# ManuelWendl/Monocular_Visual_Odometry_VA4MR

Measured on AMD Instinct MI355X. Metric: frames/s + ATE vs ref, KITTI seq00 1241x376 @ 1/2/4/8 MI355X, higher is better.
Workload: dtype mixed(u8,i32,f32,f64)

## Files before the change

### include/vo_hip.h

```cpp
#ifndef VO_HIP_H
#define VO_HIP_H
#include <stdint.h>

#ifdef __cplusplus
extern "C" {
#endif

typedef void* vo_stream_t;

enum vo_err {
    VO_OK = 0,
    VO_EARG = -1,
    VO_EHIP = -2,
};

enum vo_chain_status {
    VO_ST_OK = 0,
    VO_ST_NOT_ENOUGH_KP = 1,
    VO_ST_PNP_FAILED = 2,
    VO_ST_GFTT_NONE = 3,
    VO_ST_GFTT_ONE = 4,
    VO_ST_CAPACITY = 5,
    VO_ST_ESSENTIAL_FAILED = 6,
    VO_ST_NO_MATCHES = 7,
};

#define VO_MAX_LEVELS 8
#define VO_BORDER 16

typedef struct vo_dims {
    int32_t B, W, H;
    int32_t nlev;
    int32_t lvl_w[VO_MAX_LEVELS], lvl_h[VO_MAX_LEVELS], lvl_pitch[VO_MAX_LEVELS];
    int64_t lvl_off[VO_MAX_LEVELS];
    int64_t pyr_stride;
    int64_t der_stride;
    int32_t ncap, pcap, fcap;
    int32_t ccap;
    int32_t mcap;
    int64_t work_stride;
    int64_t iwork_stride;
} vo_dims;

typedef struct vo_opts {
    double K[9], K_inv[9];
    double min_dist_landmarks, max_dist_landmarks;
    double min_baseline_angle;
    double cos_baseline;
    int32_t min_baseline_frames;
    double feature_ratio;
    int32_t feature_max_corners;
    double feature_quality_level, feature_min_dist;
    int32_t feature_block_size, feature_use_harris;
    double harris_k;
    int32_t win_w, win_h, max_level, crit_type, crit_count;
    double crit_eps;
    double min_eig;
    double pnp_conf, pnp_error;
    int32_t pnp_iters;
} vo_opts;

typedef struct vo_state {
    uint8_t* pyr[2];
    int16_t* der[2];
// ... 237 lines not shown
```

### monocular_visual_odometry_va4mr_amd/_lib.py

```python
from __future__ import annotations

import ctypes as C
import os
import subprocess

_HERE = os.path.dirname(os.path.abspath(__file__))
LIB_PATH = os.environ.get("VO_HIP_LIB") or os.path.join(_HERE, "_build", "libvo_hip.so")
CSRC = os.path.join(_HERE, "csrc")

VO_MAX_LEVELS = 8
VO_BORDER = 16
VO_LK_USE_INITIAL_FLOW = 4
VO_LK_GET_MIN_EIGENVALS = 8
VO_LK_ILLUM_BIAS = 1
VO_LK_ILLUM_GAIN_BIAS = 2

ST_OK = 0
ST_NOT_ENOUGH_KP = 1
ST_PNP_FAILED = 2
ST_GFTT_NONE = 3
ST_GFTT_ONE = 4
ST_CAPACITY = 5
ST_ESSENTIAL_FAILED = 6
ST_NO_MATCHES = 7

STATUS_NAMES = {
    ST_OK: "ok",
    ST_NOT_ENOUGH_KP: "Not enough keypoints for PnP",
    ST_PNP_FAILED: "PnP failed",
    ST_GFTT_NONE: "goodFeaturesToTrack returned no corners",
    ST_GFTT_ONE: "goodFeaturesToTrack returned a single corner",
    ST_CAPACITY: "engine capacity exceeded",
    ST_ESSENTIAL_FAILED: "findEssentialMat found no model",
    ST_NO_MATCHES: "no bootstrap matches",
}

i32, i64, f64, vp = C.c_int32, C.c_int64, C.c_double, C.c_void_p


class VoDims(C.Structure):
    _fields_ = [
        ("B", i32), ("W", i32), ("H", i32), ("nlev", i32),
        ("lvl_w", i32 * VO_MAX_LEVELS), ("lvl_h", i32 * VO_MAX_LEVELS), ("lvl_pitch", i32 * VO_MAX_LEVELS),
        ("lvl_off", i64 * VO_MAX_LEVELS),
        ("pyr_stride", i64), ("der_stride", i64),
        ("ncap", i32), ("pcap", i32), ("fcap", i32), ("ccap", i32), ("mcap", i32),
        ("work_stride", i64), ("iwork_stride", i64),
    ]


class VoOpts(C.Structure):
    _fields_ = [
        ("K", f64 * 9), ("K_inv", f64 * 9),
        ("min_dist_landmarks", f64), ("max_dist_landmarks", f64),
        ("min_baseline_angle", f64), ("cos_baseline", f64),
        ("min_baseline_frames", i32),
        ("feature_ratio", f64),
        ("feature_max_corners", i32),
        ("feature_quality_level", f64), ("feature_min_dist", f64),
        ("feature_block_size", i32), ("feature_use_harris", i32),
        ("harris_k", f64),
        ("win_w", i32), ("win_h", i32), ("max_level", i32), ("crit_type", i32), ("crit_count", i32),
        ("crit_eps", f64), ("min_eig", f64),
        ("pnp_conf", f64), ("pnp_error", f64),
        ("pnp_iters", i32),
    ]


_STATE_FIELDS = [
    "pyr0", "pyr1", "der0", "der1", "lm_X", "lm_kp", "nL", "c_kp", "c_first", "c_tau", "nC",
# ... 142 lines not shown
```

### monocular_visual_odometry_va4mr_amd/csrc/vo_lk.hip

```cpp
#include "vo_dev.h"

#include <float.h>
#include <math.h>
#include <type_traits>

namespace {

struct LKParams {
    const uint8_t* prev;
    const int16_t* der;
    const uint8_t* next;
    int64_t pstride, dstride;
    int L;
    int lw[VO_MAX_LEVELS], lh[VO_MAX_LEVELS], lpitch[VO_MAX_LEVELS];
    int64_t loff[VO_MAX_LEVELS];
    int win_w, win_h, max_count;
    double eps2;
    float min_eig;
    float eps2_lo, eps2_hi;
    const float* p0;
    const int32_t* n0;
    int cap0;
    const float* p1;
    const int32_t* n1;
    int cap1;
    int seg1_min;
    const int32_t* chain_status;
    float* out;
    uint8_t* st;
    float* err;
    int ocap;
    const float* init;
    int eig_err;
    const float* fwd;
    double thr2;
};

VO_DEV bool lk_block(int B, int nb, int& b, int& pb, bool xcd = true, int L = -1)
{
    if (L < 0) L = blockIdx.x;
    if (B >= 8 && xcd) {
        const int xcd = L & 7, k = L >> 3;
        b = xcd + 8 * (k / nb);
        pb = k % nb;
    } else {
        b = L / nb;
        pb = L % nb;
    }
    return b < B;
}

#define LK_M 4
VO_DEV __amdgpu_buffer_rsrc_t lkq_rsrc(const void* base, int64_t bytes)
{
    return __builtin_amdgcn_make_buffer_rsrc((void*)base, (short)0, (int)bytes, 0x00020000);
}
#ifndef LK_JPRE
#define LK_JPRE 1
// ... 362 lines not shown
#endif
#ifdef VO_LK_PROF
#define LKPROF_T(var) const long long var = wall_clock64()
#else
#define LKPROF_T(var) do { } while (0)
#endif

#ifdef VO_LK_CHECK
#define LKCHK(ptr, base, bytes, what) \
    (((const char*)(ptr) >= (const char*)(base) && (const char*)(ptr) + 4 <= (const char*)(base) + (bytes)) ? true : \
     (printf("LKCHK %s b=%d p=%d level=%d off=%lld size=%lld\n", what, b, pcur, level, \
             (long long)((const char*)(ptr) - (const char*)(base)), (long long)(bytes)), false))
#else
#define LKCHK(ptr, base, bytes, what) true
#endif
#ifdef VO_LK_CHECK
#define LKCHKO(off, bytes, what) \
    do { if ((off) < 0 || (int64_t)(off) + 4 > (int64_t)(bytes)) \
        printf("LKCHK %s b=%d p=%d level=%d off=%lld size=%lld\n", what, b, pcur, level, (long long)(off), (long long)(bytes)); } while (0)
#else
#define LKCHKO(off, bytes, what) do { } while (0)
#endif

template <int WW, int WH, bool EX = false, bool ERR = true>
__global__ void __launch_bounds__(64) __attribute__((amdgpu_waves_per_eu(8, 8))) k_lk_w(LKParams P, int level_hi, int level_lo, int B, int nb, int xcd)
{
    constexpr int WPB = 1;
    constexpr int NPX = WW * WH, MAXJ = (NPX + 63) / 64;
    constexpr int TW = WW + 2 * LK_M, TH = WH + 2 * LK_M;
    constexpr int JRW = (TW + 1 + 3 + 3) / 4, IRW = (WW + 1 + 3 + 3) / 4, DRW = WW + 1;
    constexpr int QM = (TW + 3) / 4, QS = 4 * QM;
    constexpr int IRS = QS / 4, JRS = 8;
    static_assert(JRW >= QM + 1 && JRW <= JRS && IRW <= IRS && IRW <= 8 && DRW == 16 && QS % 4 == 0,
                  "k_lk_w staging layout");
    __shared__ uint4 QT4_all[WPB][(TH + 1) * QM];
    __shared__ uint32_t IR_all[WPB][(WH + 2) * IRS];
    __shared__ uint32_t DR_all[WPB][(WH + 2) * QS];
    const int wv = WPB > 1 ? (int)(threadIdx.x >> 6) : 0;
    uint4* QT4 = QT4_all[wv];
    const uint32_t* QT = reinterpret_cast<const uint32_t*>(QT4);
    uint32_t* IR = IR_all[wv];
    uint32_t* DR = DR_all[wv];
    const uint8_t* ir8 = (const uint8_t*)IR;
    int b, pb, pcur = -1;
    const int lane = lane_id();
    int level = level_lo;
    LKPROF_SET(0, wall_clock64()); LKPROF_SET(1, 0);
    for (level = level_hi; level >= level_lo; --level)
        for (int k = 2; k < 8; ++k) LKPROF_SET(k, 0);
    level = level_lo;
    if (!lk_block(B, nb, b, pb, xcd != 0, (int)blockIdx.x * WPB + wv)) return;
    if (P.chain_status && P.chain_status[b] != 0) return;
    const int n0 = P.n0 ? P.n0[b] : 0;
    int n1 = P.n1 ? P.n1[b] : 0;
    if (n1 <= P.seg1_min) n1 = 0;
    const int ntot = n0 + n1;
    const float hx = (WW - 1) * 0.5f, hy = (WH - 1) * 0.5f;
    double eps2;
    asm volatile("" : "=s"(eps2) : "0"(P.eps2));
    float eps2_lo, eps2_hi;
// ... 106 lines not shown
                    oy = __int_as_float(__builtin_amdgcn_readfirstlane(__float_as_int(P.init[2 * oidx + 1]))) * sc;
                }
            }
        }
        else if (level == level_hi) {
            ox = __int_as_float(__builtin_amdgcn_readfirstlane(__float_as_int(P.out[2 * oidx]))) * 2.f;
            oy = __int_as_float(__builtin_amdgcn_readfirstlane(__float_as_int(P.out[2 * oidx + 1]))) * 2.f;
        } else {
            ox *= 2.f;
            oy *= 2.f;
        }
        px -= hx;
        py -= hy;
        const int ipx = (int)floorf(px), ipy = (int)floorf(py);
        do {
            if ((unsigned)(ipx + WW) >= colsW || (unsigned)(ipy + WH) >= rowsW) {
                if (level == 0) { status = 0; errv = 0.f; }
                break;
            }
            bool staged = false;
            {
                LKPROF_T(ti0);
                const int gx = ipx + VO_BORDER, gy = ipy + VO_BORDER;
                const int ish = gx & 3;
                const int ln = lane;
                const int vi = loff + gy * pitch + (gx & ~3) + (ln >> 3) * pitch + 4 * (ln & 7);
                const int drow = 2 * ((ln >> 4) & 1) + (ln >> 5);
                const int vd = 4 * (loff + gy * pitch + gx + drow * pitch + (ln & 15));
                uint32_t vir[NIR], vdd[NDR], vjr[2][NJR];
#pragma unroll
                for (int k = 0; k < NIR; ++k) {
                    LKCHKO(vi + 8 * k * pitch, P.pstride, "I");
                    vir[k] = __builtin_amdgcn_raw_buffer_load_b32(rI, vi, 8 * k * pitch, 0);
                }
#pragma unroll
                for (int k = 0; k < NDR; ++k) {
                    LKCHKO(vd + 16 * k * pitch, 2 * P.dstride, "D");
                    vdd[k] = __builtin_amdgcn_raw_buffer_load_b32(rD, vd, 16 * k * pitch, 0);
                }
                {
                    const int jx = (int)floorf(ox - hx), jy = (int)floorf(oy - hy);
                    staged = LK_JPRE && (unsigned)(jx + WW) < colsW && (unsigned)(jy + WH) < rowsW && P.max_count > 0;
                    if (staged) {
                        LKPROF_ADD(3, 1);
                        j_origin(jx, jy);
                        j_issue(vjr);
                    } else {
                        tx0 = ty0 = -(1 << 28);
                    }
                }
                wave_lds_sync();
#pragma unroll
                for (int k = 0; k < NIR; ++k) {
                    const int r = (ln >> 3) + 8 * k, c = ln & 7;
                    if (c < IRS) IR[r * IRS + c] = vir[k];
                }
#pragma unroll
                for (int k = 0; k < NDR; ++k) {
                    const int r = drow + 4 * k, c = ln & 15;
                    DR[r * QS + c] = vdd[k];
                }
                if (staged) j_store(vjr);
                else wave_lds_sync();
                LKPROF_T(ti1);
                LKPROF_ADD(4, ti1 - ti0);
                float a = px - ipx, bb = py - ipy;
                const int iw00 = __float2int_rn((1.f - a) * (1.f - bb) * (float)(1 << 14));
                const int iw01 = __float2int_rn(a * (1.f - bb) * (float)(1 << 14));
                const int iw10 = __float2int_rn((1.f - a) * bb * (float)(1 << 14));
                const int iw11 = (1 << 14) - iw00 - iw01 - iw10;
                int ival[MAXJ], ixv[MAXJ], iyv[MAXJ];
                uint32_t iseed[MAXJ];
                int a11 = 0, a12 = 0, a22 = 0;
                const v2i16 wp0 = as_v2i16((uint32_t)(iw00 & 0xffff) | ((uint32_t)iw01 << 16));
                const v2i16 wp1 = as_v2i16((uint32_t)(iw10 & 0xffff) | ((uint32_t)iw11 << 16));
#pragma unroll
                for (int j = 0; j < MAXJ; ++j) {
                    const uint8_t* s = ir8 + toff[j] + ish;
                    const uint32_t* d = DR + toff[j];
                    const uint32_t d00 = d[0], d01 = d[1], d10 = d[QS], d11 = d[QS + 1];
                    const int v = DESCALE(__mul24((int)s[0], iw00) + __mul24((int)s[1], iw01) +
                                          __mul24((int)s[QS], iw10) + __mul24((int)s[QS + 1], iw11), 9);
                    const int gx2 = __builtin_amdgcn_sdot2(as_v2i16(__builtin_amdgcn_perm(d11, d10, 0x05040100u)), wp1,
                                        sdot2_sacc(__builtin_amdgcn_perm(d01, d00, 0x05040100u), v2u(wp0), 1 << 13),
                                        false) >> 14;
                    const int gy2 = __builtin_amdgcn_sdot2(as_v2i16(__builtin_amdgcn_perm(d11, d10, 0x07060302u)), wp1,
                                        sdot2_sacc(__builtin_amdgcn_perm(d01, d00, 0x07060302u), v2u(wp0), 1 << 13),
                                        false) >> 14;
                    ival[j] = v;
                    iseed[j] = 256u - ((uint32_t)ival[j] << 9);
                    ixv[j] = live[j] ? gx2 : 0;
                    iyv[j] = live[j] ? gy2 : 0;
                }
                const v2i16 gxp0 = as_v2i16(__builtin_amdgcn_perm((uint32_t)ixv[1], (uint32_t)ixv[0], 0x05040100u));
                const v2i16 gxp1 = as_v2i16(__builtin_amdgcn_perm((uint32_t)ixv[3], (uint32_t)ixv[2], 0x05040100u));
                const v2i16 gyp0 = as_v2i16(__builtin_amdgcn_perm((uint32_t)iyv[1], (uint32_t)iyv[0], 0x05040100u));
                const v2i16 gyp1 = as_v2i16(__builtin_amdgcn_perm((uint32_t)iyv[3], (uint32_t)iyv[2], 0x05040100u));
                a11 = __builtin_amdgcn_sdot2(gxp0, gxp0, sdot2_0(v2u(gxp1), v2u(gxp1)), false);
                a12 = __builtin_amdgcn_sdot2(gxp0, gyp0, sdot2_sacc(v2u(gxp1), v2u(gyp1), 1 << 24), false);
                a22 = __builtin_amdgcn_sdot2(gyp0, gyp0, sdot2_0(v2u(gyp1), v2u(gyp1)), false);
                const bool twide = __ballot(max(max((uint32_t)a11, (uint32_t)a22), (uint32_t)a12) >= (1u << 25)) != 0;
// ... 177 lines not shown
    }
    P.win_w = o->win_w;
    P.win_h = o->win_h;
    int mc = o->crit_count;
    double eps = o->crit_eps;
    if (!(o->crit_type & 1)) mc = 30;
    else mc = mc < 0 ? 0 : (mc > 100 ? 100 : mc);
    if (!(o->crit_type & 2)) eps = 0.01;
    else eps = eps < 0 ? 0 : (eps > 10 ? 10 : eps);
    P.max_count = mc;
    P.eps2 = eps * eps;
    P.min_eig = (float)o->min_eig;
    if (P.eps2 >= 0x1p-100 && P.eps2 <= 0x1p100) {
        P.eps2_lo = nextafterf((float)(P.eps2 * (1. - 0x1p-20)), 0.f);
        P.eps2_hi = nextafterf((float)(P.eps2 * (1. + 0x1p-20)), INFINITY);
    } else {
        P.eps2_lo = -INFINITY;
        P.eps2_hi = INFINITY;
    }
    P.init = nullptr;
    P.eig_err = 0;
    P.fwd = nullptr;
    P.thr2 = 0.;
}

template <bool EX, int ILL = 0>
static int launch_lk_t(const LKParams& P, int B, hipStream_t st)
{
    static_assert(EX || ILL == 0, "the illumination model lives in the EX instantiations");
    const int npx = P.win_w * P.win_h;
    if (P.win_w <= 2 || P.win_h <= 2 || P.win_w > 32 || P.win_h > 32 || npx > 64 * 16 || B < 1) return VO_EARG;
    static const int nb_env = vo_env_int("VO_LK_NB", 0);
    static const int xcd_env = vo_env_int("VO_LK_XCD", 0);
    const int nb = nb_env > 0 ? nb_env : 2048;
    const int nblk = (B >= 8 ? ((B + 7) / 8) * 8 : B) * nb;
    const int L = P.L;
    const int64_t pyr_end = P.loff[L] + (int64_t)(P.lh[L] + 2 * VO_BORDER) * P.lpitch[L];
    const bool staged15 = ILL == 0 && P.win_w == 15 && P.win_h == 15 && P.pstride >= pyr_end + 64;
    const size_t lds = 4 * (size_t)(P.win_w + 2 * LK_M) * (P.win_h + 2 * LK_M);
    if (lds > 60 * 1024) return VO_EARG;
    if (staged15) {
        if (EX || P.err) hipLaunchKernelGGL((k_lk_w<15, 15, EX>), dim3(nblk), dim3(64), 0, st, P, L, 0, B, nb, xcd_env);
        else hipLaunchKernelGGL((k_lk_w<15, 15, false, false>), dim3(nblk), dim3(64), 0, st, P, L, 0, B, nb, xcd_env);
        return hip_ok() ? VO_OK : VO_EHIP;
    }
    const bool big = P.win_w > VO_BORDER || P.win_h > VO_BORDER;
    for (int level = P.L; level >= 0; --level) {
        if (npx > 256) hipLaunchKernelGGL((k_lk<16, true, EX, ILL>), dim3(nblk), dim3(64), lds, st, P, level, B, nb);
        else if (big) hipLaunchKernelGGL((k_lk<4, true, EX, ILL>), dim3(nblk), dim3(64), lds, st, P, level, B, nb);
        else hipLaunchKernelGGL((k_lk<4, false, EX, ILL>), dim3(nblk), dim3(64), lds, st, P, level, B, nb);
    }
    return hip_ok() ? VO_OK : VO_EHIP;
}

static int launch_lk(const LKParams& P, int B, hipStream_t st) { return launch_lk_t<false>(P, B, st); }

static int launch_lk_illum(const LKParams& P, int B, hipStream_t st, int illum)
{
    if (illum == VO_LK_ILLUM_BIAS) return launch_lk_t<true, VO_LK_ILLUM_BIAS>(P, B, st);
    if (illum == VO_LK_ILLUM_GAIN_BIAS) return launch_lk_t<true, VO_LK_ILLUM_GAIN_BIAS>(P, B, st);
    return illum == 0 ? launch_lk_t<true>(P, B, st) : VO_EARG;
}

static bool lk_window_ok(const vo_opts* o)
{
// ... 187 lines not shown
```

### monocular_visual_odometry_va4mr_amd/csrc/vo_pyr.hip

```cpp
#include "vo_dev.h"

namespace {


#define PT_W 128
#define PT_H 16
#ifndef PYR0_TH
#define PYR0_TH 32
#endif
#define PV_W (PT_W + 8)
#define PV_H (PT_H + 2)
#define PS_H (2 * PV_H + 3)
#define PS_W ((2 * PV_W + 3 + 8 + 3) / 4 * 4)

struct PyrLevelArgs {
    const uint8_t* src;
    int64_t sstride;
    int sw, sh, spitch;
    int64_t soff;
    uint8_t* pyr;
    int64_t pstride;
    int16_t* der;
    int64_t dstride;
    int w, h, pitch;
// ... 165 lines not shown
                const int t0l = (ul + ll) * 3 + cl * 10;
                const int t0r = (ur + lr) * 3 + cr * 10;
                dx = t0r - t0l;
                dy = ((lr - ur) + (ll - ul)) * 3 + (lc - uc) * 10;
            }
            o[i] = (uint32_t)(uint16_t)(int16_t)dx | ((uint32_t)(uint16_t)(int16_t)dy << 16);
        }
        int16_t* dq = A.der + (int64_t)b * A.dstride + 2 * (A.off + (int64_t)py * A.pitch + px);
        *(uint4*)dq = make_uint4(o[0], o[1], o[2], o[3]);
    }
}


__global__ void __launch_bounds__(256) k_pyr01(PyrLevelArgs A0, PyrLevelArgs A1, int tx0, int ty0, int tx1)
{
    if ((int)blockIdx.y < ty0) {
        if ((int)blockIdx.x < tx0) pyr_tile<true, PYR0_TH, false>(A0, blockIdx.x * PT_W, blockIdx.y * PYR0_TH);
    } else if ((int)blockIdx.x < tx1) {
        pyr_tile<false, PT_H, true>(A1, blockIdx.x * PT_W, (blockIdx.y - ty0) * PT_H);
    }
}

#define PR_STEP 248
template <bool L0, bool RAGGED = false>
VO_DEV void pyr_rows_wave(const PyrLevelArgs& A, int R, int sx, int sy, int b)
{
    const int lane = lane_id();
    const int wo = A.w, ho = A.h;
    const int pw = wo + 2 * VO_BORDER, ph = ho + 2 * VO_BORDER;
    const int pwa = (pw + 3) & ~3;
    const int ns = (pwa + PR_STEP - 1) / PR_STEP;
    const bool lastst = sx == ns - 1;
    const int base = lastst ? max(pwa - 252, -4) : sx * PR_STEP - 4;
    const int px = base + 4 * lane;
    const int y0 = sy * R;
    if (y0 >= ho || sx >= ns) return;
    const int y1 = min(y0 + R, ho);
    const int lo = lastst ? max(pwa - PR_STEP, 0) : sx * PR_STEP;
    const int hi = lastst ? pwa : min(sx * PR_STEP + PR_STEP, pwa - PR_STEP);
    const bool wlane = lane >= 1 && lane <= 62 && px >= lo && px < hi && px < pw;
    const bool dlane = wlane && px + 3 >= VO_BORDER && px < VO_BORDER + wo;
    int fsrc[4];
#pragma unroll
    for (int j = 0; j < 4; ++j) {
        const int c = px + j;
        const int sp = (c >= 0 && c < pw) ? VO_BORDER + refl101(c - VO_BORDER, wo) : c;
        const int rel = sp - base;
// ... 8 lines not shown
            const uint32_t t = (uint32_t)__builtin_amdgcn_ds_bpermute((fsrc[j] >> 2) << 2, (int)v);
            o |= ((t >> (8 * (fsrc[j] & 3))) & 0xffu) << (8 * j);
        }
        return o;
    };
    const __amdgpu_buffer_rsrc_t rs =
        __builtin_amdgcn_make_buffer_rsrc((void*)(A.src + (int64_t)b * A.sstride), (short)0, (int)A.sstride, 0x00020000);
    uint8_t* dst = A.pyr + (int64_t)b * A.pstride + A.off;
    auto put_row = [&](int y, uint32_t v) {
        if (!wlane) return;
        *(uint32_t*)(dst + (int64_t)(VO_BORDER + y) * A.pitch + px) = v;
        if (ho >= VO_BORDER + 2) {
            if (y >= 1 && y <= VO_BORDER) *(uint32_t*)(dst + (int64_t)(VO_BORDER - y) * A.pitch + px) = v;
            if (y >= ho - 1 - VO_BORDER && y <= ho - 2)
                *(uint32_t*)(dst + (int64_t)(VO_BORDER + 2 * ho - 2 - y) * A.pitch + px) = v;
        } else {
            for (int py = 0; py < ph; ++py) {
                if (py == VO_BORDER) py = VO_BORDER + ho;
                if (py < ph && refl101(py - VO_BORDER, ho) == y) *(uint32_t*)(dst + (int64_t)py * A.pitch + px) = v;
            }
        }
    };
    auto put_der = [&](int y, uint32_t u, uint32_t c, uint32_t l) {
        const uint32_t ul = (uint32_t)__builtin_amdgcn_update_dpp(0, (int)u, 0x138, 0xF, 0xF, false);
        const uint32_t cl = (uint32_t)__builtin_amdgcn_update_dpp(0, (int)c, 0x138, 0xF, 0xF, false);
        const uint32_t ll = (uint32_t)__builtin_amdgcn_update_dpp(0, (int)l, 0x138, 0xF, 0xF, false);
        const uint32_t ur = (uint32_t)__builtin_amdgcn_update_dpp(0, (int)u, 0x130, 0xF, 0xF, false);
        const uint32_t cr = (uint32_t)__builtin_amdgcn_update_dpp(0, (int)c, 0x130, 0xF, 0xF, false);
        const uint32_t lr = (uint32_t)__builtin_amdgcn_update_dpp(0, (int)l, 0x130, 0xF, 0xF, false);
        if (!dlane || !A.der) return;
        const uint64_t U5 = ((uint64_t)u << 8) | (ul >> 24) | ((uint64_t)(ur & 0xff) << 40);
        const uint64_t L5 = ((uint64_t)l << 8) | (ll >> 24) | ((uint64_t)(lr & 0xff) << 40);
        const uint64_t C5 = ((uint64_t)c << 8) | (cl >> 24) | ((uint64_t)(cr & 0xff) << 40);
        uint32_t o[4];
#pragma unroll
        for (int i = 0; i < 4; ++i) {
            int dx = 0, dy = 0;
            const int x = px + i - VO_BORDER;
            if (x >= 0 && x < wo) {
                const int uL = (int)((U5 >> (8 * i)) & 0xff), uc = (int)((U5 >> (8 * i + 8)) & 0xff),
                          uR = (int)((U5 >> (8 * i + 16)) & 0xff);
                const int lL = (int)((L5 >> (8 * i)) & 0xff), lc = (int)((L5 >> (8 * i + 8)) & 0xff),
                          lR = (int)((L5 >> (8 * i + 16)) & 0xff);
                const int cL = (int)((C5 >> (8 * i)) & 0xff), cR = (int)((C5 >> (8 * i + 16)) & 0xff);
                dx = ((uR + lR) * 3 + cR * 10) - ((uL + lL) * 3 + cL * 10);
                dy = ((lR - uR) + (lL - uL)) * 3 + (lc - uc) * 10;
// ... 5 lines not shown
    };
    if constexpr (L0) {
        auto ld_dw = [&](int o) -> uint32_t {
            uint32_t v = __builtin_amdgcn_raw_buffer_load_b32(rs, o, 0, 0);
            if constexpr (RAGGED) {
                const int fbytes = (int)A.sstride;
                if (o < fbytes && o + 4 > fbytes) {
                    v = 0;
#pragma unroll
                    for (int k = 0; k < 3; ++k) v |= (uint32_t)(uint8_t)__builtin_amdgcn_raw_buffer_load_b8(rs, o + k, 0, 0) << (8 * k);
                }
            }
            return v;
        };
        auto ld_row = [&](int y, uint32_t& d0, uint32_t& d1) {
            const int ro = y * wo + base - VO_BORDER;
            const int al = (ro & ~3) + 4 * lane;
            d0 = ld_dw(al);
            d1 = ld_dw(al + 4);
        };
        auto val = [&](int y, uint32_t d0, uint32_t d1) {
            return fix(__builtin_amdgcn_alignbyte(d1, d0, (uint32_t)((y * wo + base - VO_BORDER) & 3)));
        };
        uint32_t a0, a1, c0, c1, n0, n1;
        const int yh = refl101(y0 - 1, ho);
        ld_row(yh, a0, a1);
        ld_row(y0, c0, c1);
        ld_row(y0 + 1 < y1 ? y0 + 1 : refl101(y1, ho), n0, n1);
        uint32_t vu = val(yh, a0, a1);
        uint32_t vc = val(y0, c0, c1);
        put_row(y0, vc);
        for (int y = y0; y < y1; ++y) {
            const int yn = y + 1 < y1 ? y + 1 : refl101(y1, ho);
            const uint32_t vl = val(yn, n0, n1);
            const int y2 = y + 2 < y1 ? y + 2 : refl101(y1, ho);
            if (y + 1 < y1) ld_row(y2, n0, n1);
            if (y + 1 < y1) put_row(y + 1, vl);
            put_der(y, vu, vc, vl);
            vu = vc;
            vc = vl;
        }
    } else {
        const int loff = 2 * px - VO_BORDER;
        auto ld_src = [&](int sr, uint32_t& d0, uint32_t& d1) {
            const int o = (int)A.soff + (VO_BORDER + sr) * A.spitch + loff;
            d0 = __builtin_amdgcn_raw_buffer_load_b32(rs, o, 0, 0);
// ... 39 lines not shown
        put_row(y0, vc);
        for (int y = y0; y < y1; ++y) {
            uint32_t vl;
            if (y + 1 < y1) {
                hx[0] = hx[2]; hy[0] = hy[2];
                hx[1] = hx[3]; hy[1] = hy[3];
                hx[2] = hx[4]; hy[2] = hy[4];
                hsum(p0, p1, hx[3], hy[3]);
                hsum(q0, q1, hx[4], hy[4]);
                ld_src(2 * y + 5, p0, p1);
                ld_src(2 * y + 6, q0, q1);
                vl = vert(hx, hy);
                put_row(y + 1, vl);
            } else {
                vl = direct(refl101(y1, ho));
            }
            put_der(y, vu, vc, vl);
            vu = vc;
            vc = vl;
        }
    }
}

template <bool L0, bool RAGGED = false>
__global__ void __launch_bounds__(64) k_pyr_rows(PyrLevelArgs A, int R)
{
    pyr_rows_wave<L0, RAGGED>(A, R, (int)blockIdx.x, (int)blockIdx.y, (int)blockIdx.z);
}

#define PYR_TAIL_MAX 6
struct PyrTailArgs {
    PyrLevelArgs a[PYR_TAIL_MAX];
    int R[PYR_TAIL_MAX];
    int n;
};
__global__ void __launch_bounds__(1024) k_pyr_tail(PyrTailArgs T)
{
    const int w = wave_id(), nw = (int)(blockDim.x >> 6);
    for (int l = 0; l < T.n; ++l) {
        const PyrLevelArgs& A = T.a[l];
        const int R = T.R[l];
        const int pwa = (A.w + 2 * VO_BORDER + 3) & ~3;
        const int ns = (pwa + PR_STEP - 1) / PR_STEP, nch = (A.h + R - 1) / R;
        for (int it = w; it < ns * nch; it += nw) pyr_rows_wave<false>(A, R, it % ns, it / ns, (int)blockIdx.x);
        __syncthreads();
    }
}

__global__ void __launch_bounds__(256) k_scharr(const uint8_t* __restrict__ pyr, int64_t pstride,
                                                int16_t* __restrict__ der, int64_t dstride,
// ... 17 lines not shown
            const int t0r = (u[px + 1] + l[px + 1]) * 3 + c[px + 1] * 10;
            const int t1l = l[px - 1] - u[px - 1], t1c = l[px] - u[px], t1r = l[px + 1] - u[px + 1];
            dx = t0r - t0l;
            dy = (t1r + t1l) * 3 + t1c * 10;
        }
        o[k] = (uint32_t)(uint16_t)(int16_t)dx | ((uint32_t)(uint16_t)(int16_t)dy << 16);
    }
    int16_t* dq = der + b * dstride + 2 * (off + (int64_t)py * pitch + px0);
    *(uint4*)dq = make_uint4(o[0], o[1], o[2], o[3]);
}

}

static bool pyr_level_args(const vo_dims* d, const vo_state* s, int cur, int l, const uint8_t* frames,
                           int64_t frame_stride, PyrLevelArgs* A)
{
    if (l == 0) {
        A->src = frames; A->sstride = frame_stride; A->sw = A->sh = A->spitch = 0; A->soff = 0;
    } else {
        A->src = s->pyr[cur]; A->sstride = d->pyr_stride;
        A->sw = d->lvl_w[l - 1]; A->sh = d->lvl_h[l - 1]; A->spitch = d->lvl_pitch[l - 1]; A->soff = d->lvl_off[l - 1];
    }
    A->pyr = s->pyr[cur]; A->pstride = d->pyr_stride;
    A->der = s->der[cur]; A->dstride = d->der_stride;
    A->w = d->lvl_w[l]; A->h = d->lvl_h[l]; A->pitch = d->lvl_pitch[l]; A->off = d->lvl_off[l];
    A->level = l;
    return A->pitch % 64 == 0 && A->pitch >= A->w + 2 * VO_BORDER;
}

extern "C" int vo_pyr_build(const vo_dims* d, const vo_state* s, int cur, const uint8_t* frames,
                            int64_t frame_stride, vo_stream_t stream)
{
    if (!d || !s || !frames || cur < 0 || cur > 1 || d->nlev < 1) return VO_EARG;
    static const int p01_env = vo_env_int("VO_PYR01", -1);
    const bool fuse01 = d->nlev >= 2 && (p01_env >= 0 ? p01_env == 1 : d->B <= 8);
    if (fuse01) {
        PyrLevelArgs A0, A1;
        if (!pyr_level_args(d, s, cur, 0, frames, frame_stride, &A0)) return VO_EARG;
        if (!pyr_level_args(d, s, cur, 1, frames, frame_stride, &A1)) return VO_EARG;
        A1.src = frames; A1.sstride = frame_stride; A1.spitch = 0; A1.soff = 0;
        const int pw0 = A0.w + 2 * VO_BORDER, ph0 = A0.h + 2 * VO_BORDER;
        const int pw1 = A1.w + 2 * VO_BORDER, ph1 = A1.h + 2 * VO_BORDER;
        const int tx0 = (pw0 + PT_W - 1) / PT_W, ty0 = (ph0 + PYR0_TH - 1) / PYR0_TH;
        const int tx1 = (pw1 + PT_W - 1) / PT_W, ty1 = (ph1 + PT_H - 1) / PT_H;
        dim3 g(tx0 > tx1 ? tx0 : tx1, ty0 + ty1, d->B);
        hipLaunchKernelGGL(k_pyr01, g, dim3(256), 0, VO_STREAM(stream), A0, A1, tx0, ty0, tx1);
    }
    static const int tail_env = vo_env_int("VO_PYR_TAIL", -1);
    const int ltail = 2;
    const bool tail = d->nlev > ltail && d->nlev - ltail <= PYR_TAIL_MAX &&
                      (tail_env >= 0 ? tail_env == 1 : d->B > 8 && d->B <= 64);
    PyrTailArgs T;
    T.n = tail ? d->nlev - ltail : 0;
    for (int i = 0; i < T.n; ++i) {
        PyrLevelArgs& A = T.a[i];
        if (!pyr_level_args(d, s, cur, ltail + i, frames, frame_stride, &A)) return VO_EARG;
        const int pwa = (A.w + 2 * VO_BORDER + 3) & ~3, ns = (pwa + PR_STEP - 1) / PR_STEP;
        const int want = ns >= 16 ? 1 : 16 / ns;
        const int R = (A.h + want - 1) / want;
        T.R[i] = R < 2 ? 2 : R;
    }
    const int lend = tail ? ltail : d->nlev;
    for (int l = fuse01 ? 2 : 0; l < lend; ++l) {
        PyrLevelArgs A;
        if (!pyr_level_args(d, s, cur, l, frames, frame_stride, &A)) return VO_EARG;
        const int pw = A.w + 2 * VO_BORDER;
        const int ns = ((pw + 3) / 4 * 4 + PR_STEP - 1) / PR_STEP;
        int R = 16;
        while (R > 4 && (int64_t)ns * ((A.h + R - 1) / R) * d->B < 8192) R >>= 1;
        dim3 g(ns, (A.h + R - 1) / R, d->B);
        if (l == 0 && (frame_stride & 3)) hipLaunchKernelGGL((k_pyr_rows<true, true>), g, dim3(64), 0, VO_STREAM(stream), A, R);
        else if (l == 0) hipLaunchKernelGGL(k_pyr_rows<true>, g, dim3(64), 0, VO_STREAM(stream), A, R);
        else hipLaunchKernelGGL(k_pyr_rows<false>, g, dim3(64), 0, VO_STREAM(stream), A, R);
    }
    if (tail) hipLaunchKernelGGL(k_pyr_tail, dim3(d->B), dim3(1024), 0, VO_STREAM(stream), T);
    return hip_ok() ? VO_OK : VO_EHIP;
}

extern "C" int vo_pyr_deriv(const vo_dims* d, const vo_state* s, int which, vo_stream_t stream)
{
    if (!d || !s || which < 0 || which > 1) return VO_EARG;
    for (int l = 0; l < d->nlev; ++l) {
        const int pw = d->lvl_w[l] + 2 * VO_BORDER, ph = d->lvl_h[l] + 2 * VO_BORDER;
        dim3 g((pw + 4 * 64 - 1) / (4 * 64), (ph + 3) / 4, d->B);
        hipLaunchKernelGGL(k_scharr, g, dim3(256), 0, VO_STREAM(stream), s->pyr[which], d->pyr_stride, s->der[which],
                           d->der_stride, d->lvl_w[l], d->lvl_h[l], d->lvl_pitch[l], d->lvl_off[l]);
    }
    return hip_ok() ? VO_OK : VO_EHIP;
}
```

### monocular_visual_odometry_va4mr_amd/engine.py

```python
from __future__ import annotations

import ctypes as C
import math
import os

import numpy as np
import torch

from . import _lib as L


def pyr_max_level(w: int, h: int, win=(15, 15), max_level: int = 3) -> int:
    sw, sh = w, h
    for lvl in range(max_level + 1):
        sw, sh = (sw + 1) // 2, (sh + 1) // 2
        if sw <= win[0] or sh <= win[1]:
            return lvl
    return max_level


def _f64_key(x: float) -> int:
    i = int(np.array([x], np.float64).view(np.int64)[0])
    return i if i >= 0 else -(i & 0x7FFFFFFFFFFFFFFF)

# ... 145 lines not shown
    eps = options.get("feature_subpix_eps")
    eps = 0.03 if eps is None else eps
    if isinstance(eps, bool) or not isinstance(eps, (int, float, np.integer, np.floating)) or \
            not (math.isfinite(eps) and eps >= 0):
        raise ValueError("feature_subpix_eps must be a finite number >= 0")
    zz = options.get("feature_subpix_zero_zone")
    zw, zh = (-1, -1) if zz is None else pair(zz, "feature_subpix_zero_zone")
    win = options.get("feature_subpix_win")
    if win is None:
        if (zw, zh) != (-1, -1) and (zw < 0 or zh < 0):
            raise ValueError("feature_subpix_zero_zone must be (-1, -1) or half sizes >= 0")
        return None
    w, h = pair(win, "feature_subpix_win")
    if not (1 <= w <= SUBPIX_MAX_HALF_WIN and 1 <= h <= SUBPIX_MAX_HALF_WIN):
        raise ValueError(f"feature_subpix_win: half-windows must be in 1..{SUBPIX_MAX_HALF_WIN}")
    if (zw, zh) != (-1, -1) and not (0 <= zw < w and 0 <= zh < h):
        raise ValueError("feature_subpix_zero_zone must be (-1, -1) or lie inside the window")
    return w, h, zw, zh, int(it), float(eps)


class Engine:

    def __init__(self, K, options: dict, width: int, height: int, batch: int = 1, device=None,
                 ncap: int = 16384, pcap: int = 16384, fcap: int = 8192):
        if not torch.cuda.is_available():
            raise RuntimeError("Engine needs a ROCm GPU (no CPU fallback)")
        self.lib = L.lib()
        self.device = torch.device(device or "cuda")
        self.K = np.asarray(K, np.float64)
        self.options = dict(options)
        self.B, self.W, self.H = int(batch), int(width), int(height)
        self.dist = parse_dist(options)
        self.K_rect = self.K
        if self.dist is not None:
            self.K = _pinhole_matrix(self.K, "K (with dist_coeffs)")
            self.K_rect = self.K if self.dist[1] is None else self.dist[1]
        self.opts = make_opts(self.K_rect, options)
        d = L.VoDims()
        d.B, d.W, d.H = self.B, self.W, self.H
        win = tuple(int(v) for v in options["winSize"])
        nlev = pyr_max_level(self.W, self.H, win, int(options["maxLevel"])) + 1
        if nlev > L.VO_MAX_LEVELS:
            raise ValueError("too many pyramid levels")
        d.nlev = nlev
        off = 0
        w, h = self.W, self.H
        pitch = ((self.W + 2 * L.VO_BORDER + 63) // 64) * 64
# ... 69 lines not shown
        self.lk_motion_model = parse_motion_model(options)
        self._seeds = self._seed_info = None
        if self.lk_motion_model is not None:
            self._seeds = z(B, ncap + pcap, 2, dt=torch.float32)
            self._seed_info = z(B, 4, dt=torch.int32)
        self.lk_illumination = parse_illumination(options)
        self._map1 = self._map2 = self._rect = None
        if self.dist is not None:
            self._map1 = torch.empty((self.H, self.W, 2), dtype=torch.int16, device=dev)
            self._map2 = torch.empty((self.H, self.W), dtype=torch.int16, device=dev)
            dc = (C.c_double * len(self.dist[0]))(*self.dist[0])
            Kc = (C.c_double * 9)(*self.K.ravel())
            Kn = None if self.dist[1] is None else (C.c_double * 9)(*self.dist[1].ravel())
            L.check(self.lib.vo_undistort_map(Kc, dc, len(dc), Kn, self.W, self.H, C.c_void_p(self._map1.data_ptr()),
                                              C.c_void_p(self._map2.data_ptr()), None, self.stream), "vo_undistort_map")
            torch.cuda.current_stream(dev).synchronize()
        self.t = T
        s = L.VoState()
        for name in L._STATE_FIELDS:
            setattr(s, name, T[name].data_ptr())
        self.state = s
        self.prev = 0
        self._pd, self._po, self._ps = C.byref(self.dims), C.byref(self.opts), C.byref(self.state)
        self._graphs = {}

    @property
    def stream(self):
        return C.c_void_p(torch.cuda.current_stream(self.device).cuda_stream)

    def _chk(self, rc, what):
        L.check(rc, what)

    def statuses(self) -> np.ndarray:
        return self.t["status"].cpu().numpy()

    def refine_info(self):
        if self._refine_info is None:
            return None
        return self._refine_info.cpu().numpy()

    def tri_gate_info(self):
        if self._tri_info is None:
            return None
        return self._tri_info.cpu().numpy()

    def seed_info(self):
# ... 72 lines not shown
        if os.environ.get("VO_ONE_STREAM") == "1":
            return torch.cuda.current_stream(self.device)
        if getattr(self, "_side", None) is None:
            hi = self.B <= 16 or self._prio_latency()
            self._side = torch.cuda.Stream(self.device, priority=-1 if hi else 0)
        return self._side

    @staticmethod
    def _prio_latency() -> bool:
        return os.environ.get("VO_PRIO_LATENCY") == "1"

    def _latency_stream(self):
        if getattr(self, "_lat", None) is None:
            self._lat = torch.cuda.Stream(self.device, priority=-1)
        return self._lat

    def _step_launch(self, frames, prev, marks=None, gftt_late=False, nxt=None):
        cur = 1 - prev
        lib = self.lib
        main = torch.cuda.current_stream(self.device)
        side = self._side_stream()
        sm, ss = C.c_void_p(main.cuda_stream), C.c_void_p(side.cuda_stream)
        pd, po, ps = self._pd, self._po, self._ps
        fp = C.c_void_p(frames.data_ptr())
        names = self.STAGES

        def run(i, strm, call):
            if marks is not None:
                marks(i, False, strm)
            self._chk(call(), "vo_" + names[i])
            if marks is not None:
                marks(i, True, strm)

        forked = side.cuda_stream != main.cuda_stream
        pre, self._pre = getattr(self, "_pre", None), None
        if pre is not None:
            main.wait_event(pre[0])
        if pre is not None and forked and pre[1] == (frames.data_ptr(), frames._version, cur) and not gftt_late:
            run(0, main, lambda: 0)
        else:
            run(0, main, lambda: lib.vo_pyr_build(pd, ps, cur, fp, self.W * self.H, sm))
        if forked:
            side.wait_stream(main)
        gftt = lambda: lib.vo_gftt(pd, po, ps, cur, ss)
        if self.feature_subpix is not None:
            sw, sh, szw, szh, sit, seps = self.feature_subpix
            seps = C.c_double(seps)

            def gftt():
                rc = lib.vo_gftt(pd, po, ps, cur, ss)
                return rc if rc != 0 else lib.vo_gftt_subpix(pd, ps, cur, sw, sh, szw, szh, sit, seps, ss)
        if not gftt_late:
            run(4, side, gftt)
        fused = getattr(self, "fuse_pnp_tri", os.environ.get("VO_PNP_TRI_SPLIT") != "1")
        defer = fused and os.environ.get("VO_COMPACT_IN_TRACK") != "1"
        track = lib.vo_track_lk if defer else lib.vo_track
        if self.lk_fb_threshold is not None:
            fb_thr, fb_scr = C.c_double(self.lk_fb_threshold), C.c_void_p(self._fb_scratch.data_ptr())
            compact = 0 if defer else 1

            def track(pd, po, ps, prev, strm):
                return lib.vo_track_fb(pd, po, ps, prev, fb_thr, fb_scr, compact, strm)
        if self.lk_motion_model is not None:
            sd, si = C.c_void_p(self._seeds.data_ptr()), C.c_void_p(self._seed_info.data_ptr())
            sd_thr = C.c_double(self.lk_fb_threshold or 0.0)
            sd_scr = None if self._fb_scratch is None else C.c_void_p(self._fb_scratch.data_ptr())
            sd_compact = 0 if defer else 1

            def track(pd, po, ps, prev, strm):
                rc = lib.vo_predict_seeds(pd, po, ps, sd, si, strm)
                return rc if rc != 0 else lib.vo_track_seeded(pd, po, ps, prev, sd, sd_thr, sd_scr, sd_compact, strm)
        if self.lk_illumination is not None:
            il = ILLUMINATION_MODELS[self.lk_illumination]
            il_sd = None if self._seeds is None else C.c_void_p(self._seeds.data_ptr())
            il_si = None if self._seed_info is None else C.c_void_p(self._seed_info.data_ptr())
            il_thr = C.c_double(self.lk_fb_threshold or 0.0)
            il_scr = None if self._fb_scratch is None else C.c_void_p(self._fb_scratch.data_ptr())
            il_compact = 0 if defer else 1

            def track(pd, po, ps, prev, strm):
                rc = 0 if il_sd is None else lib.vo_predict_seeds(pd, po, ps, il_sd, il_si, strm)
                return rc if rc != 0 else lib.vo_track_illum(pd, po, ps, prev, il, il_sd, il_thr, il_scr, il_compact, strm)
        ts = getattr(self, "track_stream", None)
        if ts is not None and forked and not gftt_late:
            ts.wait_stream(main)
            run(1, ts, lambda: track(pd, po, ps, prev, C.c_void_p(ts.cuda_stream)))
            main.wait_stream(ts)
        else:
            run(1, main, lambda: track(pd, po, ps, prev, sm))
        if gftt_late:
            run(4, side, gftt)
        ev_corners = None
        if forked:
            ev_corners = torch.cuda.Event()
            ev_corners.record(side)
        if nxt is not None and forked and not gftt_late:
            pst = side
            pst.wait_stream(main)
            nxt.record_stream(pst)
            if marks is not None:
                marks(0, False, pst)
            self._chk(lib.vo_pyr_build(pd, ps, prev, C.c_void_p(nxt.data_ptr()), self.W * self.H,
                                       C.c_void_p(pst.cuda_stream)), "vo_pyr_build")
            if marks is not None:
                marks(0, True, pst)
            ev_pre = torch.cuda.Event()
            ev_pre.record(pst)
            self._pre = (ev_pre, (nxt.data_ptr(), nxt._version, prev))
        lat = main
        if self._prio_latency() and forked:
            lat = self._latency_stream()
            lat.wait_stream(main)
        sl = C.c_void_p(lat.cuda_stream)
        if self._tri_opts is not None:
            rit, rtol = self.pnp_refine_iters, C.c_double(self.pnp_refine_ftol)
            rinfo = C.c_void_p(self._refine_info.data_ptr()) if rit else None
            tg = C.byref(self._tri_opts)
            if fused:
                pnp = lib.vo_filter_pnp_triangulate_gated if defer else lib.vo_pnp_triangulate_gated
                run(2, lat, lambda: pnp(pd, po, ps, rit, rtol, rinfo, tg, sl))
                run(3, lat, lambda: 0)
            else:
                run(2, lat, lambda: lib.vo_pnp_gated(pd, po, ps, rit, rtol, rinfo, tg, sl))
                run(3, lat, lambda: lib.vo_triangulate_gated(pd, po, ps, 0, tg, sl))
        elif self.pnp_refine_iters:
# ... 208 lines not shown
```

Baseline: 87480.

## Compute level-0 Scharr gradients on the fly in LK instead of storing them

Adds a der_first_level dims field so the pyramid builder skips writing the level-0 derivative image. The 15x15 LK kernel gains a G0 variant that loads two extra image rows and recomputes Scharr dx/dy for its patch in LDS with packed 16-bit math. This removes the full-resolution derivative write in pyramid build and the derivative reads in tracking, at the cost of extra ALU and LDS work per LK iteration tile. It is enabled automatically when the window is 15x15 and no illumination model is used.

```diff
diff --git a/include/vo_hip.h b/include/vo_hip.h
--- a/include/vo_hip.h
+++ b/include/vo_hip.h
@@ -40,6 +40,7 @@
     int32_t mcap;
     int64_t work_stride;
     int64_t iwork_stride;
+    int32_t der_first_level;
 } vo_dims;
 
 typedef struct vo_opts {
diff --git a/monocular_visual_odometry_va4mr_amd/_lib.py b/monocular_visual_odometry_va4mr_amd/_lib.py
--- a/monocular_visual_odometry_va4mr_amd/_lib.py
+++ b/monocular_visual_odometry_va4mr_amd/_lib.py
@@ -46,6 +46,7 @@
         ("pyr_stride", i64), ("der_stride", i64),
         ("ncap", i32), ("pcap", i32), ("fcap", i32), ("ccap", i32), ("mcap", i32),
         ("work_stride", i64), ("iwork_stride", i64),
+        ("der_first_level", i32),
     ]
 
 
diff --git a/monocular_visual_odometry_va4mr_amd/csrc/vo_lk.hip b/monocular_visual_odometry_va4mr_amd/csrc/vo_lk.hip
--- a/monocular_visual_odometry_va4mr_amd/csrc/vo_lk.hip
+++ b/monocular_visual_odometry_va4mr_amd/csrc/vo_lk.hip
@@ -34,6 +34,7 @@
     int eig_err;
     const float* fwd;
     double thr2;
+    int der0;
 };
 
 VO_DEV bool lk_block(int B, int nb, int& b, int& pb, bool xcd = true, int L = -1)
@@ -442,7 +443,7 @@
 #define LKCHKO(off, bytes, what) do { } while (0)
 #endif
 
-template <int WW, int WH, bool EX = false, bool ERR = true>
+template <int WW, int WH, bool EX = false, bool ERR = true, bool G0 = false>
 __global__ void __launch_bounds__(64) __attribute__((amdgpu_waves_per_eu(8, 8))) k_lk_w(LKParams P, int level_hi, int level_lo, int B, int nb, int xcd)
 {
     constexpr int WPB = 1;
@@ -454,8 +455,8 @@
     static_assert(JRW >= QM + 1 && JRW <= JRS && IRW <= IRS && IRW <= 8 && DRW == 16 && QS % 4 == 0,
                   "k_lk_w staging layout");
     __shared__ uint4 QT4_all[WPB][(TH + 1) * QM];
-    __shared__ uint32_t IR_all[WPB][(WH + 2) * IRS];
-    __shared__ uint32_t DR_all[WPB][(WH + 2) * QS];
+    __shared__ uint32_t IR_all[WPB][(WH + 2 + (G0 ? 2 : 0)) * IRS];
+    __shared__ alignas(G0 ? 16 : 4) uint32_t DR_all[WPB][(WH + 2) * QS];
     const int wv = WPB > 1 ? (int)(threadIdx.x >> 6) : 0;
     uint4* QT4 = QT4_all[wv];
     const uint32_t* QT = reinterpret_cast<const uint32_t*>(QT4);
@@ -608,21 +609,37 @@
             {
                 LKPROF_T(ti0);
                 const int gx = ipx + VO_BORDER, gy = ipy + VO_BORDER;
-                const int ish = gx & 3;
+                const bool g0 = G0 && level == 0;
+                const int gxi = g0 ? gx - 1 : gx, gyi = g0 ? gy - 1 : gy;
+                const int ish = gxi & 3;
                 const int ln = lane;
-                const int vi = loff + gy * pitch + (gx & ~3) + (ln >> 3) * pitch + 4 * (ln & 7);
+                int tl = ln;
+                if constexpr (G0) asm volatile("v_mbcnt_lo_u32_b32 %0, -1, 0\n\tv_mbcnt_hi_u32_b32 %0, -1, %0" : "=v"(tl));
+                const int vi = loff + gyi * pitch + (gxi & ~3) + (ln >> 3) * pitch + 4 * (ln & 7);
                 const int drow = 2 * ((ln >> 4) & 1) + (ln >> 5);
                 const int vd = 4 * (loff + gy * pitch + gx + drow * pitch + (ln & 15));
-                uint32_t vir[NIR], vdd[NDR], vjr[2][NJR];
-#pragma unroll
-                for (int k = 0; k < NIR; ++k) {
-                    LKCHKO(vi + 8 * k * pitch, P.pstride, "I");
-                    vir[k] = __builtin_amdgcn_raw_buffer_load_b32(rI, vi, 8 * k * pitch, 0);
-                }
-#pragma unroll
-                for (int k = 0; k < NDR; ++k) {
-                    LKCHKO(vd + 16 * k * pitch, 2 * P.dstride, "D");
-                    vdd[k] = __builtin_amdgcn_raw_buffer_load_b32(rD, vd, 16 * k * pitch, 0);
+                constexpr int NIRG = G0 ? ((WH + 3) * 8 + 63) / 64 : NIR;
+                uint32_t vir[NIRG], vdd[NDR], vjr[2][NJR];
+                if (g0) {
+                    static_assert(!G0 || (NIRG == 3 && WH + 3 == 18), "k_lk_w G0 row rounds");
+                    const int vi2 = vi + __mul24(((tl >> 3) & 1) - (tl >> 3), pitch);
+#pragma unroll
+                    for (int k = 0; k < NIRG; ++k) {
+                        const int vk = k == NIRG - 1 ? vi2 : vi;
+                        LKCHKO(vk + 8 * k * pitch, P.pstride, "I");
+                        vir[k] = __builtin_amdgcn_raw_buffer_load_b32(rI, vk, 8 * k * pitch, 0);
+                    }
+                } else {
+#pragma unroll
+                    for (int k = 0; k < NIR; ++k) {
+                        LKCHKO(vi + 8 * k * pitch, P.pstride, "I");
+                        vir[k] = __builtin_amdgcn_raw_buffer_load_b32(rI, vi, 8 * k * pitch, 0);
+                    }
+#pragma unroll
+                    for (int k = 0; k < NDR; ++k) {
+                        LKCHKO(vd + 16 * k * pitch, 2 * P.dstride, "D");
+                        vdd[k] = __builtin_amdgcn_raw_buffer_load_b32(rD, vd, 16 * k * pitch, 0);
+                    }
                 }
                 {
                     const int jx = (int)floorf(ox - hx), jy = (int)floorf(oy - hy);
@@ -636,15 +653,64 @@
                     }
                 }
                 wave_lds_sync();
-#pragma unroll
-                for (int k = 0; k < NIR; ++k) {
-                    const int r = (ln >> 3) + 8 * k, c = ln & 7;
-                    if (c < IRS) IR[r * IRS + c] = vir[k];
-                }
-#pragma unroll
-                for (int k = 0; k < NDR; ++k) {
-                    const int r = drow + 4 * k, c = ln & 15;
-                    DR[r * QS + c] = vdd[k];
+                if (g0) {
+#pragma unroll
+                    for (int k = 0; k < NIRG; ++k) {
+                        const int r = (tl >> 3) + 8 * k, c = tl & 7;
+                        if (c < IRS && r < WH + 3) IR[r * IRS + c] = vir[k];
+                    }
+                    wave_lds_sync();
+                    static_assert(DRW == 16 && WH + 1 == 16 && IRS >= 6, "k_lk_w G0 tile map");
+                    const int tr = tl >> 2, tg = tl & 3;
+                    const uint32_t* ip = IR + tr * IRS + tg;
+                    const uint32_t sel01 = 0x0c010c00u + (uint32_t)ish * 0x00010001u;
+                    const uint32_t sel23 = sel01 + 0x00020002u;
+                    v2i16 sp[3], dp[3];
+                    {
+                        const uint32_t u0 = ip[0], u1 = ip[1], u2 = ip[2];
+                        const uint32_t l0 = ip[2 * IRS], l1 = ip[2 * IRS + 1], l2 = ip[2 * IRS + 2];
+                        const v2i16 pu0 = as_v2i16(__builtin_amdgcn_perm(u1, u0, sel01)), pl0 = as_v2i16(__builtin_amdgcn_perm(l1, l0, sel01));
+                        const v2i16 pu1 = as_v2i16(__builtin_amdgcn_perm(u1, u0, sel23)), pl1 = as_v2i16(__builtin_amdgcn_perm(l1, l0, sel23));
+                        const v2i16 pu2 = as_v2i16(__builtin_amdgcn_perm(u2, u1, sel01)), pl2 = as_v2i16(__builtin_amdgcn_perm(l2, l1, sel01));
+                        sp[0] = (pu0 + pl0) * (short)3; dp[0] = pl0 - pu0;
+                        sp[1] = (pu1 + pl1) * (short)3; dp[1] = pl1 - pu1;
+                        sp[2] = (pu2 + pl2) * (short)3; dp[2] = pl2 - pu2;
+                    }
+                    {
+                        const uint32_t c0 = ip[IRS], c1 = ip[IRS + 1], c2 = ip[IRS + 2];
+                        sp[0] += as_v2i16(__builtin_amdgcn_perm(c1, c0, sel01)) * (short)10;
+                        sp[1] += as_v2i16(__builtin_amdgcn_perm(c1, c0, sel23)) * (short)10;
+                        sp[2] += as_v2i16(__builtin_amdgcn_perm(c2, c1, sel01)) * (short)10;
+                    }
+                    const v2i16 dx01 = sp[1] - sp[0], dx23 = sp[2] - sp[1];
+                    const v2i16 dm01 = as_v2i16(__builtin_amdgcn_alignbyte(v2u(dp[1]), v2u(dp[0]), 2));
+                    const v2i16 dm23 = as_v2i16(__builtin_amdgcn_alignbyte(v2u(dp[2]), v2u(dp[1]), 2));
+                    const v2i16 dy01 = (dp[1] + dp[0]) * (short)3 + dm01 * (short)10;
+                    const v2i16 dy23 = (dp[2] + dp[1]) * (short)3 + dm23 * (short)10;
+                    uint32_t o0 = __builtin_amdgcn_perm(v2u(dy01), v2u(dx01), 0x05040100u);
+                    uint32_t o1 = __builtin_amdgcn_perm(v2u(dy01), v2u(dx01), 0x07060302u);
+                    uint32_t o2 = __builtin_amdgcn_perm(v2u(dy23), v2u(dx23), 0x05040100u);
+                    uint32_t o3 = __builtin_amdgcn_perm(v2u(dy23), v2u(dx23), 0x07060302u);
+                    if (ipx < 0 || ipx + DRW > cols || ipy < 0 || ipy + WH + 1 > rows) {
+                        const bool rok = (unsigned)(ipy + tr) < (unsigned)rows;
+                        const int tx = ipx + 4 * tg;
+                        o0 = rok && (unsigned)tx < (unsigned)cols ? o0 : 0u;
+                        o1 = rok && (unsigned)(tx + 1) < (unsigned)cols ? o1 : 0u;
+                        o2 = rok && (unsigned)(tx + 2) < (unsigned)cols ? o2 : 0u;
+                        o3 = rok && (unsigned)(tx + 3) < (unsigned)cols ? o3 : 0u;
+                    }
+                    *reinterpret_cast<uint4*>(DR + tr * QS + 4 * tg) = make_uint4(o0, o1, o2, o3);
+                } else {
+#pragma unroll
+                    for (int k = 0; k < NIR; ++k) {
+                        const int r = (tl >> 3) + 8 * k, c = tl & 7;
+                        if (c < IRS) IR[r * IRS + c] = vir[k];
+                    }
+#pragma unroll
+                    for (int k = 0; k < NDR; ++k) {
+                        const int r = drow + 4 * k, c = ln & 15;
+                        DR[r * QS + c] = vdd[k];
+                    }
                 }
                 if (staged) j_store(vjr);
                 else wave_lds_sync();
@@ -660,9 +726,10 @@
                 int a11 = 0, a12 = 0, a22 = 0;
                 const v2i16 wp0 = as_v2i16((uint32_t)(iw00 & 0xffff) | ((uint32_t)iw01 << 16));
                 const v2i16 wp1 = as_v2i16((uint32_t)(iw10 & 0xffff) | ((uint32_t)iw11 << 16));
+                const int ioff = g0 ? ish + QS + 1 : ish;
 #pragma unroll
                 for (int j = 0; j < MAXJ; ++j) {
-                    const uint8_t* s = ir8 + toff[j] + ish;
+                    const uint8_t* s = ir8 + toff[j] + ioff;
                     const uint32_t* d = DR + toff[j];
                     const uint32_t d00 = d[0], d01 = d[1], d10 = d[QS], d11 = d[QS + 1];
                     const int v = DESCALE(__mul24((int)s[0], iw00) + __mul24((int)s[1], iw01) +
@@ -886,6 +953,7 @@
     P.eig_err = 0;
     P.fwd = nullptr;
     P.thr2 = 0.;
+    P.der0 = d->der_first_level;
 }
 
 template <bool EX, int ILL = 0>
@@ -903,8 +971,14 @@
     const bool staged15 = ILL == 0 && P.win_w == 15 && P.win_h == 15 && P.pstride >= pyr_end + 64;
     const size_t lds = 4 * (size_t)(P.win_w + 2 * LK_M) * (P.win_h + 2 * LK_M);
     if (lds > 60 * 1024) return VO_EARG;
+    if (P.der0 != 0 && (P.der0 != 1 || !staged15)) return VO_EARG;
     if (staged15) {
-        if (EX || P.err) hipLaunchKernelGGL((k_lk_w<15, 15, EX>), dim3(nblk), dim3(64), 0, st, P, L, 0, B, nb, xcd_env);
+        const bool err = EX || P.err;
+        if (P.der0) {
+            if (err) hipLaunchKernelGGL((k_lk_w<15, 15, EX, true, true>), dim3(nblk), dim3(64), 0, st, P, L, 0, B, nb, xcd_env);
+            else hipLaunchKernelGGL((k_lk_w<15, 15, false, false, true>), dim3(nblk), dim3(64), 0, st, P, L, 0, B, nb, xcd_env);
+        }
+        else if (err) hipLaunchKernelGGL((k_lk_w<15, 15, EX>), dim3(nblk), dim3(64), 0, st, P, L, 0, B, nb, xcd_env);
         else hipLaunchKernelGGL((k_lk_w<15, 15, false, false>), dim3(nblk), dim3(64), 0, st, P, L, 0, B, nb, xcd_env);
         return hip_ok() ? VO_OK : VO_EHIP;
     }
diff --git a/monocular_visual_odometry_va4mr_amd/csrc/vo_pyr.hip b/monocular_visual_odometry_va4mr_amd/csrc/vo_pyr.hip
--- a/monocular_visual_odometry_va4mr_amd/csrc/vo_pyr.hip
+++ b/monocular_visual_odometry_va4mr_amd/csrc/vo_pyr.hip
@@ -211,7 +211,7 @@
 }
 
 #define PR_STEP 248
-template <bool L0, bool RAGGED = false>
+template <bool L0, bool RAGGED = false, bool DER = true>
 VO_DEV void pyr_rows_wave(const PyrLevelArgs& A, int R, int sx, int sy, int b)
 {
     const int lane = lane_id();
@@ -266,6 +266,7 @@
         }
     };
     auto put_der = [&](int y, uint32_t u, uint32_t c, uint32_t l) {
+        if constexpr (!DER) return;
         const uint32_t ul = (uint32_t)__builtin_amdgcn_update_dpp(0, (int)u, 0x138, 0xF, 0xF, false);
         const uint32_t cl = (uint32_t)__builtin_amdgcn_update_dpp(0, (int)c, 0x138, 0xF, 0xF, false);
         const uint32_t ll = (uint32_t)__builtin_amdgcn_update_dpp(0, (int)l, 0x138, 0xF, 0xF, false);
@@ -317,6 +318,18 @@
         auto val = [&](int y, uint32_t d0, uint32_t d1) {
             return fix(__builtin_amdgcn_alignbyte(d1, d0, (uint32_t)((y * wo + base - VO_BORDER) & 3)));
         };
+        if constexpr (!DER) {
+            for (int y = y0; y < y1; y += 4) {
+                uint32_t d0[4], d1[4];
+#pragma unroll
+                for (int k = 0; k < 4; ++k)
+                    if (y + k < y1) ld_row(y + k, d0[k], d1[k]);
+#pragma unroll
+                for (int k = 0; k < 4; ++k)
+                    if (y + k < y1) put_row(y + k, val(y + k, d0[k], d1[k]));
+            }
+            return;
+        }
         uint32_t a0, a1, c0, c1, n0, n1;
         const int yh = refl101(y0 - 1, ho);
         ld_row(yh, a0, a1);
@@ -402,10 +415,10 @@
     }
 }
 
-template <bool L0, bool RAGGED = false>
+template <bool L0, bool RAGGED = false, bool DER = true>
 __global__ void __launch_bounds__(64) k_pyr_rows(PyrLevelArgs A, int R)
 {
-    pyr_rows_wave<L0, RAGGED>(A, R, (int)blockIdx.x, (int)blockIdx.y, (int)blockIdx.z);
+    pyr_rows_wave<L0, RAGGED, DER>(A, R, (int)blockIdx.x, (int)blockIdx.y, (int)blockIdx.z);
 }
 
 #define PYR_TAIL_MAX 6
@@ -469,7 +482,7 @@
         A->sw = d->lvl_w[l - 1]; A->sh = d->lvl_h[l - 1]; A->spitch = d->lvl_pitch[l - 1]; A->soff = d->lvl_off[l - 1];
     }
     A->pyr = s->pyr[cur]; A->pstride = d->pyr_stride;
-    A->der = s->der[cur]; A->dstride = d->der_stride;
+    A->der = l < d->der_first_level ? nullptr : s->der[cur]; A->dstride = d->der_stride;
     A->w = d->lvl_w[l]; A->h = d->lvl_h[l]; A->pitch = d->lvl_pitch[l]; A->off = d->lvl_off[l];
     A->level = l;
     return A->pitch % 64 == 0 && A->pitch >= A->w + 2 * VO_BORDER;
@@ -479,6 +492,7 @@
                             int64_t frame_stride, vo_stream_t stream)
 {
     if (!d || !s || !frames || cur < 0 || cur > 1 || d->nlev < 1) return VO_EARG;
+    if (d->der_first_level < 0 || d->der_first_level > 1) return VO_EARG;
     static const int p01_env = vo_env_int("VO_PYR01", -1);
     const bool fuse01 = d->nlev >= 2 && (p01_env >= 0 ? p01_env == 1 : d->B <= 8);
     if (fuse01) {
@@ -516,7 +530,10 @@
         int R = 16;
         while (R > 4 && (int64_t)ns * ((A.h + R - 1) / R) * d->B < 8192) R >>= 1;
         dim3 g(ns, (A.h + R - 1) / R, d->B);
-        if (l == 0 && (frame_stride & 3)) hipLaunchKernelGGL((k_pyr_rows<true, true>), g, dim3(64), 0, VO_STREAM(stream), A, R);
+        const bool ragged = (frame_stride & 3) != 0;
+        if (l == 0 && !A.der && ragged) hipLaunchKernelGGL((k_pyr_rows<true, true, false>), g, dim3(64), 0, VO_STREAM(stream), A, R);
+        else if (l == 0 && !A.der) hipLaunchKernelGGL((k_pyr_rows<true, false, false>), g, dim3(64), 0, VO_STREAM(stream), A, R);
+        else if (l == 0 && ragged) hipLaunchKernelGGL((k_pyr_rows<true, true>), g, dim3(64), 0, VO_STREAM(stream), A, R);
         else if (l == 0) hipLaunchKernelGGL(k_pyr_rows<true>, g, dim3(64), 0, VO_STREAM(stream), A, R);
         else hipLaunchKernelGGL(k_pyr_rows<false>, g, dim3(64), 0, VO_STREAM(stream), A, R);
     }
@@ -527,7 +544,8 @@
 extern "C" int vo_pyr_deriv(const vo_dims* d, const vo_state* s, int which, vo_stream_t stream)
 {
     if (!d || !s || which < 0 || which > 1) return VO_EARG;
-    for (int l = 0; l < d->nlev; ++l) {
+    if (d->der_first_level < 0 || d->der_first_level > 1) return VO_EARG;
+    for (int l = d->der_first_level; l < d->nlev; ++l) {
         const int pw = d->lvl_w[l] + 2 * VO_BORDER, ph = d->lvl_h[l] + 2 * VO_BORDER;
         dim3 g((pw + 4 * 64 - 1) / (4 * 64), (ph + 3) / 4, d->B);
         hipLaunchKernelGGL(k_scharr, g, dim3(256), 0, VO_STREAM(stream), s->pyr[which], d->pyr_stride, s->der[which],
diff --git a/monocular_visual_odometry_va4mr_amd/engine.py b/monocular_visual_odometry_va4mr_amd/engine.py
--- a/monocular_visual_odometry_va4mr_amd/engine.py
+++ b/monocular_visual_odometry_va4mr_amd/engine.py
@@ -191,7 +191,7 @@
 class Engine:
 
     def __init__(self, K, options: dict, width: int, height: int, batch: int = 1, device=None,
-                 ncap: int = 16384, pcap: int = 16384, fcap: int = 8192):
+                 ncap: int = 16384, pcap: int = 16384, fcap: int = 8192, lk_grad0=None):
         if not torch.cuda.is_available():
             raise RuntimeError("Engine needs a ROCm GPU (no CPU fallback)")
         self.lib = L.lib()
@@ -307,6 +307,16 @@
         self.state = s
         self.prev = 0
         self._pd, self._po, self._ps = C.byref(self.dims), C.byref(self.opts), C.byref(self.state)
+        pyr_end = d.lvl_off[nlev - 1] + (d.lvl_h[nlev - 1] + 2 * L.VO_BORDER) * d.lvl_pitch[nlev - 1]
+        eligible = win == (15, 15) and self.lk_illumination is None and d.pyr_stride >= pyr_end + 64
+        if lk_grad0 is not None and not isinstance(lk_grad0, (bool, np.bool_)):
+            raise ValueError("lk_grad0 must be None (automatic), True or False")
+        if lk_grad0 and not eligible:
+            raise ValueError("lk_grad0 needs winSize (15, 15) and no lk_illumination (the 15x15 LK kernel)")
+        self.lk_grad0 = eligible if lk_grad0 is None else bool(lk_grad0)
+        self.dims_step = L.VoDims.from_buffer_copy(self.dims)
+        self.dims_step.der_first_level = 1 if self.lk_grad0 else 0
+        self._pd_step = C.byref(self.dims_step)
         self._graphs = {}
 
     @property
@@ -425,6 +435,7 @@
         side = self._side_stream()
         sm, ss = C.c_void_p(main.cuda_stream), C.c_void_p(side.cuda_stream)
         pd, po, ps = self._pd, self._po, self._ps
+        pds = self._pd_step
         fp = C.c_void_p(frames.data_ptr())
         names = self.STAGES
 
@@ -442,7 +453,7 @@
         if pre is not None and forked and pre[1] == (frames.data_ptr(), frames._version, cur) and not gftt_late:
             run(0, main, lambda: 0)
         else:
-            run(0, main, lambda: lib.vo_pyr_build(pd, ps, cur, fp, self.W * self.H, sm))
+            run(0, main, lambda: lib.vo_pyr_build(pds, ps, cur, fp, self.W * self.H, sm))
         if forked:
             side.wait_stream(main)
         gftt = lambda: lib.vo_gftt(pd, po, ps, cur, ss)
@@ -487,10 +498,10 @@
         ts = getattr(self, "track_stream", None)
         if ts is not None and forked and not gftt_late:
             ts.wait_stream(main)
-            run(1, ts, lambda: track(pd, po, ps, prev, C.c_void_p(ts.cuda_stream)))
+            run(1, ts, lambda: track(pds, po, ps, prev, C.c_void_p(ts.cuda_stream)))
             main.wait_stream(ts)
         else:
-            run(1, main, lambda: track(pd, po, ps, prev, sm))
+            run(1, main, lambda: track(pds, po, ps, prev, sm))
         if gftt_late:
             run(4, side, gftt)
         ev_corners = None
@@ -503,7 +514,7 @@
             nxt.record_stream(pst)
             if marks is not None:
                 marks(0, False, pst)
-            self._chk(lib.vo_pyr_build(pd, ps, prev, C.c_void_p(nxt.data_ptr()), self.W * self.H,
+            self._chk(lib.vo_pyr_build(pds, ps, prev, C.c_void_p(nxt.data_ptr()), self.W * self.H,
                                        C.c_void_p(pst.cuda_stream)), "vo_pyr_build")
             if marks is not None:
                 marks(0, True, pst)
```

Result: no change. 88320 (median of 6 runs) (+1.0%).
